# norabelrose/sparse-vae

Measured on AMD Instinct MI355X. Metric: training tokens/sec + ELBO match vs CPU ref, 512-tok seq, 1/2/4/8 MI355X, higher is better.
Workload: dtype bf16; 1 GPU; c2: TransformerVAE 6L d512 heads 8 seq 512, batch 64/GPU, dense attention, dropout 0.1, fwd+bwd+allreduce+clip+RAdam; model=TransformerVAE-6L-d512, global_batch=64, seq_len=512, parallelism=dp1

## Files before the change

### include/svae.h

```cpp
#ifndef SVAE_H
#define SVAE_H
#include <stdint.h>
#ifdef __cplusplus
extern "C" {
#endif

typedef void* svae_stream_t;

enum svae_epi {
  SVAE_EPI_BF16 = 0,
  SVAE_EPI_F32 = 1,
  SVAE_EPI_F32_ACC = 2,
  SVAE_EPI_F32_ATOMIC = 3,
  SVAE_EPI_GELU = 4,
  SVAE_EPI_GELU_BWD = 5,
  SVAE_EPI_DROPOUT_RESID = 6,
  SVAE_EPI_ROTARY_BF16 = 7,
  SVAE_EPI_CE_STATS = 8,
  SVAE_EPI_CE_PROB = 9,
  SVAE_EPI_ROWSCALE_GATHER = 10
};

typedef struct svae_gemm_desc {
  const void* A;
// ... 43 lines not shown
                      const float* zrows, int32_t zmod, const float* w, const float* b, float* xo, void* h, float* mean,
                      float* rstd, int32_t rows, int32_t D, svae_stream_t stream);
int svae_layernorm_fwd(const void* x, int32_t x_dtype, const float* w, const float* b, void* y,
                       float* mean, float* rstd, int32_t rows, int32_t D, svae_stream_t stream);
int svae_layernorm_bwd(const void* dy, const void* x, int32_t x_dtype, const float* w, const float* mean,
                       const float* rstd, const float* dres, float* dx, void* dx_bf, float* part,
                       int32_t nblk, int32_t rows, int32_t D, int32_t zero_mod, svae_stream_t stream);
int svae_layernorm_bwd_drop(const void* dy, const void* x, int32_t x_dtype, const float* w, const float* mean,
                            const float* rstd, const float* dres, float* dx, void* dx_bf, float* part, int32_t nblk,
                            int32_t rows, int32_t D, int32_t zero_mod, float bf_drop_p, uint64_t bf_seed,
                            int32_t bf_zero_mod, float* zrow, void* zrow_bf, svae_stream_t stream);
int svae_layernorm_bwd_gelu(const void* dy, const void* x, int32_t x_dtype, const float* w, const float* mean,
                            const float* rstd, const void* gp, void* out_bf, float* part, int32_t nblk, int32_t rows,
                            int32_t D, svae_stream_t stream);
int svae_layernorm_fwd_z(float* x, const float* zrows, int32_t zmod, const float* w, const float* b, void* y,
                         float* mean, float* rstd, int32_t rows, int32_t D, svae_stream_t stream);
int svae_layernorm_nblk(int32_t rows);
#define SVAE_LN_MULTI_MAX 4
int svae_layernorm_fwd_multi(const float* x, const float* const* w, const float* const* b, void* const* y, int32_t n,
                             float* mean, float* rstd, int32_t rows, int32_t D, svae_stream_t stream);
int svae_layernorm_bwd_multi(const void* const* dy, const float* x, const float* const* w, const float* mean,
                             const float* rstd, const float* dres, float* dx, float* const* part, int32_t nblk,
                             int32_t n, int32_t rows, int32_t D, svae_stream_t stream);

int svae_colsum(const void* in, int32_t in_dtype, int32_t rows, int32_t cols, int64_t ld, float* out,
                int32_t accumulate, svae_stream_t stream);

#define SVAE_COLSUM_MAX 8
typedef struct svae_colsum_seg {
  const float* in;
  float* out;
  int64_t ld;
  int32_t rows, cols;
} svae_colsum_seg;
int svae_colsum_multi(const svae_colsum_seg* segs, int32_t n, svae_stream_t stream);

typedef struct svae_attn_desc {
  const void* q; const void* k; const void* v; void* o;
  int64_t sq, sk, sv, so, bq, bk, bv, bo;
  const uint8_t* key_pad;
  float* lse;
  int32_t B, H, Lq, Lk, hd, causal;
  float scale;
  const void* dout; int64_t sdo, bdo;
  float* delta;
  float* dq;
// ... 247 lines not shown
```

### sparse-vae_amd/csrc/layernorm.hip

```cpp
#include <algorithm>

#include "common.h"
#include "../../include/svae.h"

using namespace svae;

namespace {


template <typename T>
__device__ __forceinline__ f32x4 load4(const T* p);
template <>
__device__ __forceinline__ f32x4 load4<float>(const float* p) { return *(const f32x4*)p; }
template <>
__device__ __forceinline__ f32x4 load4<bf16>(const bf16* p) {
  bf16x4 v = *(const bf16x4*)p;
  return (f32x4){(float)v[0], (float)v[1], (float)v[2], (float)v[3]};
}
__device__ __forceinline__ void store4_bf(bf16* p, f32x4 v) {
  *(bf16x4*)p = (bf16x4){f2bf(v[0]), f2bf(v[1]), f2bf(v[2]), f2bf(v[3])};
}

template <int MAXV>
__device__ __forceinline__ int ln_col(int lane, int k) {
// ... 426 lines not shown
    const float m1 = wave_sum(s1) / D, m2 = wave_sum(s2) / D;
#pragma unroll
    for (int j = 0; j < MAXV; ++j) {
      const int c = (lane + 64 * j) * 4;
      if (c < D) {
        f32x4 o;
#pragma unroll
        for (int e = 0; e < 4; ++e) o[e] = rstd * (g[j][e] - m1 - xh[j][e] * m2) + cur.rr[j][e];
        *(f32x4*)(dx + base + c) = o;
      }
    }
    cur = nxt;
  }
#pragma unroll
  for (int i = 0; i < NM; ++i) {
    if (i >= m.n) break;
    if (i > 0) __syncthreads();
#pragma unroll
    for (int j = 0; j < MAXV; ++j) {
      const int c = (lane + 64 * j) * 4;
      if (c < D) {
        *(f32x4*)&red[wave][0][c] = adw[i][j];
        *(f32x4*)&red[wave][1][c] = adb[i][j];
      }
    }
    __syncthreads();
    for (int c = threadIdx.x; c < 2 * D; c += 256) {
      const int which = c / D, col = c % D;
      const float s = red[0][which][col] + red[1][which][col] + red[2][which][col] + red[3][which][col];
      m.part[i][((long long)blockIdx.x * 2 + which) * D + col] = s;
    }
  }
}

template <typename T>
__global__ __launch_bounds__(256) void colsum_kernel(const T* __restrict__ in, int rows, int cols, long long ld,
                                                     float* __restrict__ out, int rows_per_split) {
  __shared__ f32x4 red[16][17];
  const int ct = threadIdx.x & 15, rt = threadIdx.x >> 4;
  const int c = (blockIdx.x * 16 + ct) * 4;
  const int r0 = blockIdx.y * rows_per_split;
  const int r1 = min(rows, r0 + rows_per_split);
  f32x4 acc = {0.f, 0.f, 0.f, 0.f};
  if (c < cols) {
    int r = r0 + rt;
    for (; r + 112 < r1; r += 128) {
// ... 196 lines not shown
  SVAE_LAUNCH_CHECK();
  return SVAE_OK;
}

SVAE_EXPORT int svae_layernorm_bwd_multi(const void* const* dy, const float* x, const float* const* w, const float* mean,
                                         const float* rstd, const float* dres, float* dx, float* const* part,
                                         int32_t nblk, int32_t n, int32_t rows, int32_t D, svae_stream_t stream) {
  if (!dy || !x || !w || !mean || !rstd || !dx || !part || n <= 0 || n > SVAE_LN_MULTI_MAX || rows <= 0 || D <= 0 ||
      D % 4 || D > 1024 || nblk <= 0)
    return SVAE_EINVAL;
  LnMulti m = {};
  m.n = n;
  for (int i = 0; i < n; ++i) {
    if (!dy[i] || !w[i] || !part[i]) return SVAE_EINVAL;
    m.dy[i] = (const bf16*)dy[i]; m.w[i] = w[i]; m.part[i] = part[i];
  }
  hipStream_t s = (hipStream_t)stream;
#define SVAE_LN_BWDM(MV) \
  hipLaunchKernelGGL((ln_bwd_multi_kernel<MV>), dim3(nblk), dim3(256), 0, s, m, x, mean, rstd, dres, dx, rows, D)
  if (D <= 512) SVAE_LN_BWDM(2);
  else if (D <= 768) SVAE_LN_BWDM(3);
  else SVAE_LN_BWDM(4);
#undef SVAE_LN_BWDM
  SVAE_LAUNCH_CHECK();
  return SVAE_OK;
}

SVAE_EXPORT int svae_layernorm_nblk(int32_t rows) {
  int n = (rows + 3) / 4;
  return n < 1024 ? n : 1024;
}

SVAE_EXPORT int svae_layernorm_bwd_drop(const void* dy, const void* x, int32_t x_dtype, const float* w,
                                        const float* mean, const float* rstd, const float* dres, float* dx, void* dx_bf,
                                        float* part, int32_t nblk, int32_t rows, int32_t D, int32_t zero_mod,
                                        float bf_drop_p, uint64_t bf_seed, int32_t bf_zero_mod, float* zrow,
                                        void* zrow_bf, svae_stream_t stream) {
  if (!dy || !x || !w || !mean || !rstd || !dx || !part || rows <= 0 || D <= 0 || D % 4 || D > 1024 || nblk <= 0)
    return SVAE_EINVAL;
  if (bf_drop_p < 0.f || bf_drop_p >= 1.f || ((bf_drop_p > 0.f || bf_zero_mod > 0) && !dx_bf)) return SVAE_EINVAL;
  if ((zrow || zrow_bf) && zero_mod <= 0) return SVAE_EINVAL;
  hipStream_t s = (hipStream_t)stream;
#define SVAE_LN_BWD(MV)                                                                                            \
  do {                                                                                                             \
    if (x_dtype == 0)                                                                                              \
      hipLaunchKernelGGL((ln_bwd_kernel<float, MV>), dim3(nblk), dim3(256), 0, s, (const bf16*)dy, (const float*)x, \
// ... 65 lines not shown
```

### sparse-vae_amd/sparse_vae/_native.py

```python
import ctypes
import os

import torch

_HERE = os.path.dirname(os.path.abspath(__file__))
LIB_PATH = os.environ.get('SVAE_LIB') or os.path.join(_HERE, 'libsvae.so')

c_void_p, c_int32, c_int64, c_float, c_uint64 = (ctypes.c_void_p, ctypes.c_int32, ctypes.c_int64,
                                                  ctypes.c_float, ctypes.c_uint64)
c_fptr = ctypes.c_void_p

EPI_BF16, EPI_F32, EPI_F32_ACC, EPI_F32_ATOMIC, EPI_GELU, EPI_GELU_BWD, EPI_DROPOUT_RESID, \
    EPI_ROTARY_BF16, EPI_CE_STATS, EPI_CE_PROB, EPI_ROWSCALE_GATHER = range(11)

LATENT_L2, LATENT_COSINE, LATENT_KL = range(3)
LATENT_METRICS = {'l2': LATENT_L2, 'cosine': LATENT_COSINE, 'kl': LATENT_KL}
LATENT_MAX_BLOCKS = 1024
TSNE_ROWS_PER_BLOCK, TSNE_TILE_COLS = 512, 256
PAIR_RBF, PAIR_IMQ = range(2)
PAIR_KINDS = {'rbf': PAIR_RBF, 'imq': PAIR_IMQ}
PAIRSUM_TILE_COLS, PAIRSUM_MAX_P, MMD_REDUCE_BLOCKS = 32, 8, 256
KMEANS_MAX_K, KMEANS_TILE_CENTROIDS, KMEANS_SORT_BLOCKS, KMEANS_SEED_BLOCK_ROWS = 1024, 32, 256, 256
TEXT_MAX_LEN = 2048
BEAM_MAX_W = 16
# ... 25 lines not shown
        ('q', c_void_p), ('k', c_void_p), ('v', c_void_p), ('o', c_void_p),
        ('sq', c_int64), ('sk', c_int64), ('sv', c_int64), ('so', c_int64),
        ('bq', c_int64), ('bk', c_int64), ('bv', c_int64), ('bo', c_int64),
        ('key_pad', c_void_p), ('lse', c_void_p),
        ('B', c_int32), ('H', c_int32), ('Lq', c_int32), ('Lk', c_int32), ('hd', c_int32), ('causal', c_int32),
        ('scale', c_float),
        ('dout', c_void_p), ('sdo', c_int64), ('bdo', c_int64),
        ('delta', c_void_p), ('dq', c_void_p), ('bdq', c_int64),
        ('dk', c_void_p), ('dv', c_void_p),
        ('sdk', c_int64), ('sdv', c_int64), ('bdk', c_int64), ('bdv', c_int64),
        ('rot_tab', c_void_p), ('rot_d', c_int32),
        ('o32', c_void_p), ('so32', c_int64), ('bo32', c_int64),
        ('dq_part', c_void_p), ('dq_bf', c_void_p), ('ldq_bf', c_int64),
        ('window', c_int32),
        ('delta_ready', c_int32),
        ('o_lo', c_void_p), ('so_lo', c_int64), ('bo_lo', c_int64),
        ('fwd_ws', c_void_p), ('fwd_ws_elems', c_int64),
    ]


GROUP_MAX = 256
COLSUM_MAX = 8
LN_MULTI_MAX = 4


ZPROJ_MAX = 32


class ZprojSeg(ctypes.Structure):
    _fields_ = [('g', c_void_p), ('W', c_void_p), ('dW', c_void_p), ('db', c_void_p)]


class ZprojFwdSeg(ctypes.Structure):
    _fields_ = [('W', c_void_p), ('bias', c_void_p), ('out', c_void_p)]


class ColsumSeg(ctypes.Structure):
    _fields_ = [('inp', c_void_p), ('out', c_void_p), ('ld', c_int64), ('rows', c_int32), ('cols', c_int32)]


_SIGS = {
    'svae_gemm': [ctypes.POINTER(GemmDesc), c_void_p],
    'svae_gemm_pair': [ctypes.POINTER(GemmDesc), ctypes.POINTER(GemmDesc), c_void_p],
    'svae_gemm_group_table_bytes': [c_int32],
    'svae_gemm_group': [ctypes.POINTER(GemmDesc), c_int32, c_int32, c_void_p, c_void_p, c_int64, c_void_p],
    'svae_resid_ln_fwd': [c_void_p, c_void_p, c_int32, c_int64, c_float, c_uint64, c_void_p, c_int32, c_void_p,
# ... 32 lines not shown
    'svae_ce_label_logit': [c_void_p, c_int64, c_void_p, c_int64, c_void_p, c_void_p, c_int32, c_int32, c_void_p,
                            c_void_p],
    'svae_ce_prob_finalize': [c_void_p, c_int32, c_void_p, c_void_p, c_int32, c_int32, c_int32, c_int32, c_void_p,
                              c_void_p, c_void_p, c_void_p, c_void_p, c_void_p],
    'svae_ce_prob_finalize_fix': [c_void_p, c_int32, c_void_p, c_void_p, c_int32, c_int32, c_int32, c_int32, c_void_p,
                                  c_void_p, c_void_p, c_void_p, c_void_p, c_void_p, c_int64, c_void_p, c_int64, c_void_p,
                                  c_void_p, c_int64, c_int32, c_int32, c_void_p, c_void_p],
    'svae_ce_prob_bwd_prep': [c_void_p, c_int64, c_void_p, c_void_p, c_void_p, c_void_p, c_void_p, c_int32, c_int32,
                              c_int32, c_int32, c_int32, c_void_p, c_void_p, c_void_p, c_void_p, c_void_p],
    'svae_embedding_bwd_ce': [c_void_p, c_void_p, c_void_p, c_int32, c_int32, c_int32, c_void_p, c_void_p, c_void_p],
    'svae_ce_grad': [c_void_p, c_int64, c_void_p, c_void_p, c_void_p, c_void_p, c_void_p, c_int32, c_int32, c_int32,
                     c_int32, c_int32, c_void_p],
    'svae_dropout_bwd_cast': [c_void_p, c_void_p, c_float, c_uint64, c_int64, c_int32, c_int64, c_void_p],
    'svae_gelu_bwd': [c_void_p, c_void_p, c_void_p, c_int64, c_void_p],
    'svae_prep_tokens': [c_void_p, c_void_p, c_int32, c_int32, c_int32, c_void_p, c_void_p, c_void_p, c_void_p,
                         c_void_p, c_void_p],
    'svae_step_scalars': [c_void_p, c_void_p, c_void_p, c_float, c_void_p, c_void_p, c_void_p],
    'svae_zproj_bwd_multi': [c_void_p, c_int32, c_void_p, c_void_p, c_int32, c_int32, c_int32, c_void_p],
    'svae_zproj_fwd_multi': [c_void_p, c_int32, c_void_p, c_int32, c_int32, c_int32, c_void_p],
    'svae_layernorm_fwd_multi': [c_void_p, c_void_p, c_void_p, c_void_p, c_int32, c_void_p, c_void_p, c_int32, c_int32,
                                 c_void_p],
    'svae_layernorm_bwd_multi': [c_void_p, c_void_p, c_void_p, c_void_p, c_void_p, c_void_p, c_void_p, c_void_p,
                                 c_int32, c_int32, c_int32, c_int32, c_void_p],
    'svae_layernorm_fwd_z': [c_void_p, c_void_p, c_int32, c_void_p, c_void_p, c_void_p, c_void_p, c_void_p, c_int32,
                             c_int32, c_void_p],
    'svae_cast_bf16': [c_void_p, c_void_p, c_int64, c_void_p],
    'svae_extract_rows': [c_void_p, c_int64, c_int32, c_int32, c_int32, c_void_p, c_void_p],
    'svae_zproj_bwd': [c_void_p, c_void_p, c_void_p, c_void_p, c_void_p, c_void_p, c_int32, c_int32, c_int32, c_void_p],
    'svae_sumsq': [c_void_p, c_int64, c_void_p, c_int32, c_void_p],
    'svae_radam': [c_void_p, c_void_p, c_void_p, c_void_p, c_void_p, c_int64, c_void_p, c_int32, c_void_p,
                   c_void_p, c_void_p],
    'svae_gemm_f32': [c_void_p, c_void_p, c_void_p, c_int32, c_int32, c_int32, c_int64, c_int64, c_int64, c_void_p,
                      c_void_p, c_int64, c_int32, c_void_p, c_int32, c_int32, c_int32, c_void_p],
    'svae_attn_fwd_f32': [c_void_p, c_void_p, c_void_p, c_void_p, c_int64, c_int64, c_int64, c_int64, c_int64, c_int64,
                          c_int64, c_int64, c_void_p, c_int32, c_int32, c_int32, c_int32, c_int32, c_int32, c_int32,
                          c_float, c_void_p],
    'svae_layernorm_fwd_f32': [c_void_p, c_void_p, c_void_p, c_void_p, c_int32, c_int32, c_void_p],
    'svae_ce_seq_logprob': [c_void_p, c_int32, c_void_p, c_void_p, c_int32, c_int32, c_void_p, c_void_p],
    'svae_dec_linear': [c_void_p, c_int64, c_void_p, c_int64, c_void_p, c_void_p, c_int64, c_void_p, c_int64, c_int32,
                        c_int32, c_int32, c_int32, c_void_p, c_int32, c_int32, c_void_p, c_void_p, c_int64, c_void_p],
    'svae_dec_attn': [c_void_p, c_int64, c_void_p, c_void_p, c_int32, c_int32, c_int32, c_int32, c_void_p, c_int32,
                      c_float, c_void_p, c_int64, c_void_p],
    'svae_dec_embed': [c_void_p, c_int32, c_void_p, c_void_p, c_void_p, c_int32, c_int32, c_void_p],
    'svae_dec_penalty': [c_void_p, c_int64, c_int32, c_void_p, c_void_p, c_int32, c_void_p, c_void_p, c_float,
                         c_void_p],
    'svae_dec_sample': [c_void_p, c_int64, c_int32, c_int32, c_void_p, c_void_p, c_int32, c_void_p, c_void_p, c_int32,
# ... 98 lines not shown
```

### sparse-vae_amd/sparse_vae/engine.py

```python
import math
import os
from collections import OrderedDict

import torch

from . import kernels as K
from ._native import COLSUM_MAX, GROUP_MAX, LN_MULTI_MAX, ZPROJ_MAX
from ._native import EPI_BF16, EPI_F32, EPI_F32_ACC, EPI_GELU, EPI_GELU_BWD, EPI_DROPOUT_RESID, \
    EPI_ROTARY_BF16, EPI_CE_STATS, EPI_F32_ATOMIC, EPI_CE_PROB, EPI_ROWSCALE_GATHER

bf16, f32 = torch.bfloat16, torch.float32
ALIGN = 64
CE_CHUNK_NUMEL = 2 ** 30


def _attn_entries(pre, d, learned):
    out = []
    if learned:
        out.append((pre + 'learned_queries', (1, learned, d)))
        names = ['k_linear', 'v_linear']
    else:
        names = ['q_linear', 'k_linear', 'v_linear']
    out += [(pre + n + '.weight', (d, d)) for n in names]
    out += [(pre + n + '.bias', (d,)) for n in names]
    out += [(pre + 'output_linear.weight', (d, d)), (pre + 'output_linear.bias', (d,))]
    return out


def _ctx_ln_entries(pre, d):
    return [(pre + 'context_layer_norm.weight', (d,)), (pre + 'context_layer_norm.bias', (d,))]
# ... 260 lines not shown

    def _bname(self, name, st):
        return f'{name}.{st["tag"]}' if self._dw_names else name

    def flush_dw(self):
        q, self._dw_jobs = self._dw_jobs, []
        k = 0
        for c in range(0, len(q), GROUP_MAX):
            jobs = q[c:c + GROUP_MAX]
            key = tuple((j.n_out, j.n_in, j.rows) for j in jobs)
            if key not in self._dwg_sched:
                self._dwg_sched[key] = K.group_schedule(key, self.ncu)
            for idx, splits, slab in self._dwg_sched[key]:
                if len(self._dwg_states) <= k:
                    self._dwg_states.append(K.DwGroupState(self.P.device))
                K.linear_dw_group([jobs[i] for i in idx], splits, self._dwg_states[k], slab=slab)
                k += 1

    def _db(self, dY, bname, rows, cols, ld=None):
        off = self.P.offsets[bname][0]
        K.colsum(dY, rows, cols, ld or cols, self.P.grad[off:off + cols])

    def layer_fwd(self, pre, x, B, Sx, L, pad, *, learned=0, cross=False, causal=False, ctx=None, heads, hd,
                  drop_p=0.0, seed=0, tag, out=None, window=0, out_bf=None, zsplice=None, ctx_ln=None):
        d, ws, P = self.d, self.ws, self.P
        rows_x = B * Sx
        rot = self.rot(max(Sx, L), window)
        st = {'pre': pre, 'B': B, 'Sx': Sx, 'L': L, 'learned': learned, 'cross': cross, 'causal': causal,
              'heads': heads, 'hd': hd, 'drop_p': drop_p, 'seed': seed, 'x': x, 'tag': tag, 'window': window}
        a = pre + 'attention.'
        h, st['ln_a'] = self._ln_fwd(pre + 'attn_layer_norm', x, rows_x, tag + '.ln_a', zsplice=zsplice)
        st['h'] = h
        pad_k = pad if Sx == L else None
        if learned:
            Lq = learned
            kv = ws.get(tag + '.kv', (rows_x, 2 * d))
            K.gemm(h, P.w(a + 'k_linear.weight'), kv, rows_x, 2 * d, d, epi=EPI_ROTARY_BF16,
                   bias=P.f(a + 'k_linear.bias'), rot=rot, rot_cols=d, rot_d=d, rot_seq=Sx)
            q = P.w(a + 'learned_queries').view(Lq, d)
            qargs = dict(sq=d, bq=0)
            kt, vt, sk = kv, kv[:, d:], 2 * d
            st['kv'] = kv
        else:
            Lq = Sx
            qkv = ws.get(tag + '.qkv', (rows_x, 3 * d))
            K.gemm(h, P.w(a + 'q_linear.weight'), qkv, rows_x, 3 * d, d, epi=EPI_ROTARY_BF16,
                   bias=P.f(a + 'q_linear.bias'), rot=rot, rot_cols=2 * d, rot_d=d, rot_seq=Sx)
            q = qkv
            qargs = dict(sq=3 * d, bq=Sx * 3 * d)
            kt, vt, sk = qkv[:, d:], qkv[:, 2 * d:], 3 * d
            st['qkv'] = qkv
        rows_q = B * Lq
        O = ws.get(tag + '.O', (rows_q, d))
        Ox = self._o_extra(tag + '.O', rows_q, d, Lq)
# ... 34 lines not shown
                   bias=P.f(c + 'output_linear.bias'), resid=x1, ldr=d)
            st.update(cx=cx, hq=hq, qc=qc, kvc=kvc, Oc=Oc, lsec=lsec, x2=x2, pad_ctx=pad)
            xc = x2
        h2, st['ln_f'] = self._ln_fwd(pre + 'ffn_layer_norm', xc, rows_q, tag + '.ln_f')
        gprime = ws.get(tag + '.gprime', (rows_q, 4 * d))
        f = ws.get(tag + '.f', (rows_q, 4 * d))
        K.gemm(h2, P.w(pre + 'ffn.0.weight'), f, rows_q, 4 * d, d, epi=EPI_GELU, bias=P.f(pre + 'ffn.0.bias'),
               aux=gprime, ldaux=4 * d)
        out = ws.get(tag + '.out', (rows_q, d), f32) if out is None else out
        K.gemm(f, P.w(pre + 'ffn.2.weight'), out, rows_q, d, 4 * d, epi=EPI_DROPOUT_RESID, resid=xc, ldr=d,
               drop_p=drop_p, seed=seed, aux=out_bf, ldaux=d if out_bf is not None else 0)
        st.update(h2=h2, gprime=gprime, f=f, xc=xc, rows_q=rows_q)
        return out, st

    def _o_extra(self, tag, rows_q, d, Lq):
        return dict(o_lo=self.ws.get(tag + 'lo', (rows_q, d)), so_lo=d, bo_lo=Lq * d)

    def _dq_part(self, B, H, Lq, Lk, hd, window=0):
        n = K.attn_dq_part_elems(B, H, Lq, Lk, hd, window)
        t = self.ws.bufs.get('b.dqpart')
        return t if t is not None and t.numel() >= n else self.ws.get('b.dqpart', (n,), f32)

    def layer_bwd(self, st, dout, dx_out, *, dx_accumulate=False, dctx=None, g2_ready=False, next_drop=None,
                  zsplice=None, next_st=None):
        d, ws, P = self.d, self.ws, self.P
        pre, B, Sx, L, Lq = st['pre'], st['B'], st['Sx'], st['L'], st['Lq']
        heads, hd = st['heads'], st['hd']
        rows_x, rows_q = B * Sx, st['rows_q']
        rot = self.rot(max(Sx, L), st['window'])
        a = pre + 'attention.'
        bn = lambda name: self._bname(name, st)
        self._dwq = self._dw_jobs if self._dw_names else None
        g2 = ws.get(bn('b.g2'), (rows_q, d))
        if not g2_ready:
            K.dropout_bwd_cast(dout, g2, st['drop_p'], st['seed'], rows_q, d)
        dpre = ws.get(bn('b.dpre'), (rows_q, 4 * d))
        K.gemm(g2, P.wT(pre + 'ffn.2.weight', d, 4 * d), dpre, rows_q, 4 * d, d, epi=EPI_GELU_BWD, aux=st['gprime'],
               ldaux=4 * d)
        self._dw_pair(self._job(g2, st['f'], pre + 'ffn.2.weight', rows_q, d, 4 * d),
                      self._job(dpre, st['h2'], pre + 'ffn.0.weight', rows_q, 4 * d, d, bias=pre + 'ffn.0.bias'))
        dh2 = ws.get('b.dh2', (rows_q, d))
        K.gemm(dpre, P.wT(pre + 'ffn.0.weight', 4 * d, d), dh2, rows_q, d, 4 * d, epi=EPI_BF16)
        dxc = ws.get('b.dxc', (rows_q, d), f32)
        gxc = ws.get(bn('b.gxc'), (rows_q, d))
        self._ln_bwd(pre + 'ffn_layer_norm', dh2, st['ln_f'], rows_q, dout, dxc, gxc)
        dx1, gx1 = dxc, gxc
        if st['cross']:
# ... 43 lines not shown
                                           bias=a + 'k_linear.bias'))
            dh = ws.get('b.dh', (rows_x, d))
            K.gemm(dkv, P.wT(a + 'k_linear.weight', 2 * d, d), dh, rows_x, d, 2 * d, epi=EPI_BF16)
        else:
            qkv = st['qkv']
            dqkv = ws.get(bn('b.dqkv'), (rows_x, 3 * d))
            K.attention(qkv, qkv[:, d:], qkv[:, 2 * d:], st['O'], st['lse'], B=B, H=heads, Lq=Lq, Lk=Sx, hd=hd,
                        sq=3 * d, bq=Sx * 3 * d, sk=3 * d, sv=3 * d, bk=Sx * 3 * d, bv=Sx * 3 * d, so=d, bo=Lq * d,
                        key_pad=st['pad_k'], causal=st['causal'], window=st['window'], backward=True, dout=dO,
                        sdo=d, bdo=Lq * d, delta=delta, dq_bf=dqkv, ldq_bf=3 * d, dk=dqkv[:, d:], dv=dqkv[:, 2 * d:],
                        sdk=3 * d, sdv=3 * d, bdk=Sx * 3 * d, bdv=Sx * 3 * d, rot=rot, rot_d=d, **st['Ox'],
                        dq_part=self._dq_part(B, heads, Lq, Sx, hd, st['window']))
            self._dw_pair(wo_dw, self._job(dqkv, st['h'], a + 'q_linear.weight', rows_x, 3 * d, d,
                                           bias=a + 'q_linear.bias'))
            dh = ws.get('b.dh', (rows_x, d))
            K.gemm(dqkv, P.wT(a + 'q_linear.weight', 3 * d, d), dh, rows_x, d, 3 * d, epi=EPI_BF16)
        if st['resid']:
            self._ln_bwd(pre + 'attn_layer_norm', dh, st['ln_a'], rows_x, dx1, dx_out,
                         dx_bf=(ws.get(self._bname('b.g2', next_st or st), (rows_x, d)) if next_drop is not None
                                else None), bf_drop=next_drop,
                         zsplice=zsplice)
            if dx_accumulate:
                raise NotImplementedError('residual + accumulate is handled by the caller')
        else:
            self._ln_bwd(pre + 'attn_layer_norm', dh, st['ln_a'], rows_x, dx_out if dx_accumulate else None, dx_out)
        self._dwq = None

    def forward(self, ids, ntok, *, pad=True, eps=None, seed=0, kl_weight=1.0, dropout=0.1, need_logits=False):
        hp, d, ws, P = self.hp, self.d, self.ws, self.P
        if not ids.is_cuda:
            raise RuntimeError('VAEEngine needs device tensors (no CPU fallback)')
        P.sync_shadow()
        B, L = ids.shape
        T, V, Z, N = B * L, hp.vocab_size, hp.latent_depth, hp.num_latents
        ids32 = ws.get('ids', (B, L), torch.int32)
        padm = None
        if pad is not None and pad is not False:
            padm = ws.get('pad', (B, L), torch.uint8)
        labels = ws.get('labels', (B, L), torch.int32)
        ntok64 = ws.get('ntok', (B,), torch.int64)
        if (ids.dtype == torch.int64 and ids.is_contiguous() and isinstance(ntok, torch.Tensor) and ntok.is_cuda
                and ntok.dtype == torch.int64 and ntok.is_contiguous() and ntok.numel() == B
                and (padm is None or pad is True or (pad.dtype == torch.bool and pad.is_contiguous()))):
            K.prep_tokens(ids, pad if padm is not None else None, B, L, ids32, labels, padm, ntok, ntok64)
        else:
            ids32, padm = self._inputs(ids, pad)
            labels[:, :-1].copy_(ids32[:, 1:])
            labels[:, -1] = 0
            ntok64.copy_(ntok)
        sv = {'B': B, 'L': L, 'dropout': dropout, 'seed': seed}

        x_emb = ws.get('x_emb', (T, d), f32)
        K.embedding_fwd(ids32, P.f('input_layer.0.weight'), x_emb, T, d, out2=ws.get('x_dec0', (T, d), f32))

        enc_bf, stats, sv['enc_layers'] = self._encode(x_emb, B, L, padm, dropout, seed)

        zf = ws.get('z', (B, Z), f32)
        zb = ws.get('z_bf', (B, Z))
        eps_buf = ws.get('eps', (B, Z), f32)
        raw_kl = ws.get('raw_kl', (B,), f32)
        kl = ws.get('kl', (2,), f32)
        if eps is not None:
            eps_buf.copy_(eps.reshape(B, Z))
        K.reparam_fwd(stats, eps_buf if eps is not None else None, _mix_seed(seed, 7), ntok64, zf, zb, eps_buf,
                      raw_kl, kl, B, Z)
        sv.update(enc_bf=enc_bf, stats=stats, z_bf=zb, eps=eps_buf)

        xf, sv['dec_layers'] = self._decode(x_emb, zb, padm, B, L, dropout, seed, x_ready=True)

        hh, gp0, h0, ln_h = self._head_hidden(xf, T)
        nchunks, chunk_len = K.ce_chunking(B, L, V, CE_CHUNK_NUMEL)
        lse = ws.get('ce.lse', (T,), f32)
        row_loss = ws.get('ce.row_loss', (T,), f32)
        chunk_w = ws.get('ce.chunk_w', (max(8, nchunks),), f32)
        nll = ws.get('nll', (1,), f32)
        ntile = -(-V // 128)
        head = 'logits' if need_logits else self.head_mode
        W, bias = P.w('input_layer.0.weight'), P.f('output_layer.3.bias')
# ... 20 lines not shown
            sat = ws.get('ce.sat', (T + 1,), torch.int32)
            K.ce_prob_finalize(part, ntile, coff, labels, T, L, nchunks, chunk_len, lse, row_loss, chunk_w, nll,
                               fix=(hh, W, bias, logits, sat))
        else:
            K.ce_finalize(part, ntile, lab_logit, labels, T, L, nchunks, chunk_len, lse, row_loss, chunk_w, nll)
        sv.update(xf=xf, gp0=gp0, h0=h0, hh=hh, ln_h=ln_h, logits=logits, lse=lse, chunk_w=chunk_w,
                  nchunks=nchunks, chunk_len=chunk_len, labels=labels, ids32=ids32, ntok=ntok64, x_emb=x_emb,
                  row_loss=row_loss, head=head, coff=coff)
        loss = ws.get('loss', (1,), f32)
        K.step_scalars(kl_weight, nll=nll, kl=kl, loss=loss)
        self.saved = sv
        return {'loss': loss[0], 'nll': nll[0], 'kl': kl[0], 'train_kl': kl[1], 'raw_kl': raw_kl,
                'mu': stats[:, :Z], 'logvar': stats[:, Z:], 'stats': stats, 'kl_buf': kl, 'z': zf, 'eps': eps_buf,
                'logits': logits if need_logits else None,
                'ce_saturated': sat[0] if head == 'prob' else None}

    def weighted_nll(self, tok_w):
        sv = self.saved
        out = torch.empty(1, dtype=f32, device=self.P.device)
        B, L = sv['B'], sv['L']
        K.ce_weighted_nll(sv['row_loss'], sv['labels'], tok_w, B * L, L, sv['nchunks'], sv['chunk_len'], out)
        return out[0]

    def _encode(self, x_emb, B, L, padm, dropout, seed):
        hp, d, ws, P = self.hp, self.d, self.ws, self.P
        N, Z = hp.num_latents, hp.latent_depth
        lay = []
        z, st = self.layer_fwd('encoder.first_layer.', x_emb, B, L, L, padm, learned=N, heads=self.He, hd=64,
                               drop_p=dropout, seed=_mix_seed(seed, 1000), tag='e0')
        lay.append(st)
        nmid = hp.enc_layers - 2
        cxs = self._ctx_ln_fwd(x_emb, B * L, nmid) if P.ctx_batched else [None] * nmid
        for j in range(nmid):
            z, st = self.layer_fwd(f'encoder.middle_layers.{j}.', z, B, N, L, padm, cross=True, ctx=x_emb,
                                   heads=self.He, hd=64, drop_p=dropout, seed=_mix_seed(seed, 1001 + j), tag=f'e{j + 1}',
                                   ctx_ln=cxs[j])
            lay.append(st)
        enc, st = self.layer_fwd('encoder.bottleneck.', z, B, N, L, padm, learned=1, heads=self.He, hd=64,
                                 drop_p=dropout, seed=_mix_seed(seed, 1999), tag='eb')
        lay.append(st)
        enc_bf = ws.get('enc_bf', (B, d))
        K.cast_bf16(enc, enc_bf)
        stats = ws.get('stats', (B, 2 * Z), f32)
        K.gemm(enc_bf, P.w('q_of_z_given_x.linear.weight'), stats, B, 2 * Z, d, epi=EPI_F32,
               bias=P.f('q_of_z_given_x.linear.bias'))
        return enc_bf, stats, lay

    def _ctx_ln_fwd(self, x, rows, nmid):
        D, ws, P = self.d, self.ws, self.P
        mean = ws.get('ctx.ln.mean', (rows,), f32)
        rstd = ws.get('ctx.ln.rstd', (rows,), f32)
        out = []
        for j0 in range(0, nmid, LN_MULTI_MAX):
            js = range(j0, min(nmid, j0 + LN_MULTI_MAX))
            names = [f'encoder.middle_layers.{j}.context_layer_norm' for j in js]
# ... 273 lines not shown
                self._zp_pending.append((dzh_i, P.w(wz), P.g(wz), P.g(bz)))
            else:
                self.flush_zproj()
                K.extract_rows(dx_prev, d, T, L, d, dzh)
                K.cast_bf16(dzh, dzh_bf)
                self._dw(self._job(dzh_bf, sv['z_bf'], wz, B, d, Z, bias=bz))
                K.gemm(dzh_bf, P.w(wz), dz, B, Z, d, b_t=True, epi=EPI_F32_ATOMIC, splits=max(1, min(8, d // 64)))
            ready(P.end(f'z_projections.{i}.bias'))
            dx, dx_prev = dx_prev, dx
        self.flush_zproj()
        dx_emb = dx

        dstats = ws.get('b.dstats', (B, 2 * Z), f32)
        K.reparam_bwd(sv['stats'], sv['eps'], dz, sv['ntok'], gs[1:2], dstats, B, Z)
        dstats_bf = ws.get('b.dstats_bf', (B, 2 * Z))
        K.cast_bf16(dstats, dstats_bf)
        self._dw(self._job(dstats_bf, sv['enc_bf'], 'q_of_z_given_x.linear.weight', B, 2 * Z, d))
        self._db(dstats, 'q_of_z_given_x.linear.bias', B, 2 * Z)
        denc = ws.get('b.denc', (B, d), f32)
        K.gemm(dstats_bf, P.w('q_of_z_given_x.linear.weight'), denc, B, d, 2 * Z, b_t=True, epi=EPI_F32)
        ready(P.end('q_of_z_given_x.linear.bias'))

        enc = sv['enc_layers']
        dcur = denc
        for k in reversed(range(1, len(enc))):
            st = enc[k]
            nxt = ws.get(f'b.denc{k}', (B * N, d), f32)
            self.layer_bwd(st, dcur, nxt, dctx=dx_emb)
            ready(P.end(st['pre'] + 'ffn_layer_norm.bias'))
            dcur = nxt
        deferred = [st for st in enc if st.get('ctx_deferred')]
        if deferred:
            self._ctx_ln_bwd(deferred[::-1], dx_emb)
            ready(P.end(deferred[0]['pre'] + 'context_layer_norm.bias'))
        st0 = enc[0]
        if st0['resid']:
            tmp = ws.get('b.dfirst', (T, d), f32)
            self.layer_bwd(st0, dcur, tmp)
            self.flush_dw()
            K.embedding_bwd(sv['ids32'], tmp, P.g('input_layer.0.weight'), T, d)
        else:
            self.layer_bwd(st0, dcur, dx_emb, dx_accumulate=True)
            self.flush_dw()

        ready(P.end('encoder.first_layer.ffn_layer_norm.bias'))
        self._embedding_bwd(sv, dx_emb, T, d)
        ready(P.n_live)
        self.flush_colsum()

    def _embedding_bwd(self, sv, dx, T, d):
        if sv['head'] == 'prob':
            K.embedding_bwd_ce(sv['ids32'], dx, self.P.g('input_layer.0.weight'), T, d, sv['L'], sv['hh'], sv['ce_q'])
        else:
            K.embedding_bwd(sv['ids32'], dx, self.P.g('input_layer.0.weight'), T, d)
```

### sparse-vae_amd/sparse_vae/kernels.py

```python
import ctypes
import os
from typing import NamedTuple

import torch

from . import _native as N
from ._native import lib, check, ptr, stream

bf16, f32 = torch.bfloat16, torch.float32

_gemm_desc = N.GemmDesc()


def _dev(*ts):
    for t in ts:
        if t is not None and not t.is_cuda:
            raise RuntimeError('libsvae kernels need device tensors (no CPU fallback)')


def gemm(A, B, C, M, N_, K, *, a_t=False, b_t=False, lda=None, ldb=None, ldc=None, epi=N.EPI_BF16, bias=None,
         resid=None, ldr=0, aux=None, ldaux=0, alpha=1.0, splits=1, drop_p=0.0, seed=0, rot=None, rot_cols=0,
         rot_d=0, rot_seq=0, labels=None, label_logit=None, batch=1, sA=0, sB=0, sC=0, a_rowsum=None, k_weight=None,
         row_a=None, row_b=None, gather=None, ldg=0, delta=None, delta_o32=None, ld_o32=0, delta_hd=0, delta_seq=0):
    d = _fill_desc(_gemm_desc, A, B, C, M, N_, K, a_t=a_t, b_t=b_t, lda=lda, ldb=ldb, ldc=ldc, epi=epi, bias=bias,
# ... 279 lines not shown

def _ptrs(ts):
    return (ctypes.c_void_p * N.LN_MULTI_MAX)(*[t.data_ptr() for t in ts])


def layernorm_fwd_multi(x, ws, bs, ys, mean, rstd, rows, D):
    n = len(ys)
    assert 0 < n <= N.LN_MULTI_MAX and len(ws) == n and len(bs) == n and x.dtype == f32
    _dev(x, mean, rstd, *ws, *bs, *ys)
    check(lib.svae_layernorm_fwd_multi(x.data_ptr(), _ptrs(ws), _ptrs(bs), _ptrs(ys), n, mean.data_ptr(),
                                       rstd.data_ptr(), rows, D, stream()), 'svae_layernorm_fwd_multi')


def layernorm_bwd_multi(dys, x, ws, mean, rstd, dres, dx, wgrads, rows, D, part_ws, defer=None):
    n = len(dys)
    assert 0 < n <= N.LN_MULTI_MAX and len(ws) == n and len(wgrads) == n and x.dtype == f32
    _dev(x, mean, rstd, dx, *dys, *ws)
    nblk = lib.svae_layernorm_nblk(rows)
    parts = [part_ws[j * nblk * 2 * D:(j + 1) * nblk * 2 * D] for j in range(n)]
    assert parts[-1].numel() == nblk * 2 * D
    check(lib.svae_layernorm_bwd_multi(_ptrs(dys), x.data_ptr(), _ptrs(ws), mean.data_ptr(), rstd.data_ptr(),
                                       ptr(dres), dx.data_ptr(), _ptrs(parts), nblk, n, rows, D, stream()),
          'svae_layernorm_bwd_multi')
    for part, wg in zip(parts, wgrads):
        if defer is not None:
            defer.append((part, nblk, 2 * D, 2 * D, wg))
        else:
            colsum(part, nblk, 2 * D, 2 * D, wg, accumulate=True)


_colsum_segs = (N.ColsumSeg * N.COLSUM_MAX)()


def colsum_multi(segs):
    assert 0 < len(segs) <= N.COLSUM_MAX
    for i, (inp, rows, cols, ld, out) in enumerate(segs):
        _dev(inp, out)
        assert inp.dtype == f32 and out.dtype == f32
        _colsum_segs[i].inp, _colsum_segs[i].out = inp.data_ptr(), out.data_ptr()
        _colsum_segs[i].ld, _colsum_segs[i].rows, _colsum_segs[i].cols = ld, rows, cols
    check(lib.svae_colsum_multi(ctypes.addressof(_colsum_segs), len(segs), stream()), 'svae_colsum_multi')


def colsum(inp, rows, cols, ld, out, accumulate=True):
    check(lib.svae_colsum(inp.data_ptr(), 0 if inp.dtype == f32 else 1, rows, cols, ld, out.data_ptr(),
                          int(accumulate), stream()), 'svae_colsum')
# ... 817 lines not shown
```

Baseline: 2.826 million tokens/s.

## Fuse embedding gather with encoder layernorms in forward and backward

Adds a kernel that gathers embedding rows and in one pass computes the shared layernorm statistics and writes the bf16 normalized outputs for the first layer's attention LN and the middle layers' context LNs. A matching backward kernel folds those layernorm backwards, including weight/bias partial sums, into the embedding scatter-add. This removes separate embedding and LN launches and extra round trips of the T×d activations through memory. In exchange it adds more complex gradient-readiness ordering for the allreduce and per-element atomics into the embedding table in the fused backward.

```diff
diff --git a/include/svae.h b/include/svae.h
--- a/include/svae.h
+++ b/include/svae.h
@@ -89,6 +89,14 @@
 int svae_layernorm_bwd_multi(const void* const* dy, const float* x, const float* const* w, const float* mean,
                              const float* rstd, const float* dres, float* dx, float* const* part, int32_t nblk,
                              int32_t n, int32_t rows, int32_t D, svae_stream_t stream);
+#define SVAE_EMB_LN_MAX (SVAE_LN_MULTI_MAX + 1)
+int svae_embedding_ln_fwd_multi(const int32_t* ids, const void* table, const float* const* w, const float* const* b,
+                                void* const* y, int32_t n, float* out, float* out2, float* mean, float* rstd,
+                                int32_t rows, int32_t D, svae_stream_t stream);
+int svae_embedding_bwd_ln_multi(const int32_t* ids, const float* dx, const float* x, const float* mean,
+                                const float* rstd, const void* const* dy, const float* const* w, float* const* part,
+                                int32_t nblk, int32_t n, float* dtable, int32_t rows, int32_t D, int32_t seq,
+                                const void* hh, const float* q, svae_stream_t stream);
 
 int svae_colsum(const void* in, int32_t in_dtype, int32_t rows, int32_t cols, int64_t ld, float* out,
                 int32_t accumulate, svae_stream_t stream);
diff --git a/sparse-vae_amd/csrc/layernorm.hip b/sparse-vae_amd/csrc/layernorm.hip
--- a/sparse-vae_amd/csrc/layernorm.hip
+++ b/sparse-vae_amd/csrc/layernorm.hip
@@ -472,6 +472,166 @@
       if (c < D) {
         *(f32x4*)&red[wave][0][c] = adw[i][j];
         *(f32x4*)&red[wave][1][c] = adb[i][j];
+      }
+    }
+    __syncthreads();
+    for (int c = threadIdx.x; c < 2 * D; c += 256) {
+      const int which = c / D, col = c % D;
+      const float s = red[0][which][col] + red[1][which][col] + red[2][which][col] + red[3][which][col];
+      m.part[i][((long long)blockIdx.x * 2 + which) * D + col] = s;
+    }
+  }
+}
+
+struct EmbLn {
+  const float* w[SVAE_EMB_LN_MAX];
+  const float* b[SVAE_EMB_LN_MAX];
+  bf16* y[SVAE_EMB_LN_MAX];
+  const bf16* dy[SVAE_EMB_LN_MAX];
+  float* part[SVAE_EMB_LN_MAX];
+  int n;
+};
+
+template <int MAXV>
+__global__ __launch_bounds__(256) void emb_ln_fwd_multi_kernel(const int* __restrict__ ids,
+                                                               const float* __restrict__ table, EmbLn m,
+                                                               float* __restrict__ out, float* __restrict__ out2,
+                                                               float* __restrict__ mean_out,
+                                                               float* __restrict__ rstd_out, int rows, int D) {
+  const int lane = threadIdx.x & 63;
+  const int nw = gridDim.x * 4;
+  int row = blockIdx.x * 4 + (threadIdx.x >> 6);
+  if (row >= rows) return;
+  f32x4 v[MAXV], vn[MAXV];
+  ln_load_row<float, MAXV>(table + (long long)ids[row] * D, lane, D, v);
+#pragma nounroll
+  while (true) {
+    const int next = row + nw;
+    if (next < rows) ln_load_row<float, MAXV>(table + (long long)ids[next] * D, lane, D, vn);
+#pragma unroll
+    for (int k = 0; k < MAXV; ++k) {
+      const int c = ln_col<MAXV>(lane, k);
+      if (c < D) {
+        *(f32x4*)(out + (long long)row * D + c) = v[k];
+        *(f32x4*)(out2 + (long long)row * D + c) = v[k];
+      }
+    }
+    float s = 0.f;
+#pragma unroll
+    for (int k = 0; k < MAXV; ++k) s += (v[k][0] + v[k][1]) + (v[k][2] + v[k][3]);
+    const float mean = wave_sum(s) / D;
+    float sq = 0.f;
+#pragma unroll
+    for (int k = 0; k < MAXV; ++k) {
+      const bool in = ln_col<MAXV>(lane, k) < D;
+#pragma unroll
+      for (int e = 0; e < 4; ++e) { const float t = in ? v[k][e] - mean : 0.f; sq += t * t; }
+    }
+    const float rstd = rsqrtf(wave_sum(sq) / D + 1e-5f);
+#pragma unroll
+    for (int j = 0; j < SVAE_EMB_LN_MAX; ++j)
+      if (j < m.n) ln_store_row<MAXV>(v, mean, rstd, m.w[j], m.b[j], m.y[j] + (long long)row * D, lane, D);
+    if (lane == 0) { mean_out[row] = mean; rstd_out[row] = rstd; }
+    if (next >= rows) break;
+    for (int k = 0; k < MAXV; ++k) v[k] = vn[k];
+    row = next;
+  }
+}
+
+template <int NK, int NM>
+__global__ __launch_bounds__(256) void emb_bwd_ln_multi_kernel(const int* __restrict__ ids, EmbLn m,
+                                                               const float* __restrict__ dx,
+                                                               const float* __restrict__ x,
+                                                               const float* __restrict__ mean_in,
+                                                               const float* __restrict__ rstd_in,
+                                                               float* __restrict__ dtable, int rows, int D, int seq,
+                                                               const bf16* __restrict__ hh,
+                                                               const float* __restrict__ q) {
+  __shared__ float red[4][2][64 * NK];
+  const int lane = threadIdx.x & 63, wave = threadIdx.x >> 6;
+  float adw[NM][NK], adb[NM][NK];
+#pragma unroll
+  for (int i = 0; i < NM; ++i)
+#pragma unroll
+    for (int k = 0; k < NK; ++k) { adw[i][k] = 0.f; adb[i][k] = 0.f; }
+  struct RowIn {
+    float xv[NK], rr[NK];
+    bf16 dv[NM][NK], hv[NK];
+    float mean, rstd, qp;
+    long long dst;
+  };
+  auto load_row = [&](int row, RowIn& in) {
+    const long long base = (long long)row * D;
+    in.mean = mean_in[row];
+    in.rstd = rstd_in[row];
+    in.dst = (long long)ids[row] * D;
+    const bool head = hh && row % seq != 0;
+    in.qp = head ? q[row - 1] : 0.f;
+#pragma unroll
+    for (int k = 0; k < NK; ++k) {
+      const int c = lane + 64 * k;
+      const bool ok = c < D;
+      in.xv[k] = ok ? x[base + c] : 0.f;
+      in.rr[k] = ok ? dx[base + c] : 0.f;
+      in.hv[k] = ok && head ? hh[base - D + c] : (bf16)0.f;
+#pragma unroll
+      for (int i = 0; i < NM; ++i) {
+        if (i >= m.n) break;
+        in.dv[i][k] = ok ? m.dy[i][base + c] : (bf16)0.f;
+      }
+    }
+  };
+  const int stride = gridDim.x * 4;
+  int row = blockIdx.x * 4 + wave;
+  RowIn cur, nxt;
+  if (row < rows) load_row(row, cur);
+  for (; row < rows; row += stride) {
+    if (row + stride < rows) load_row(row + stride, nxt);
+    const float mean = cur.mean, rstd = cur.rstd, qp = cur.qp;
+    const long long dst = cur.dst;
+    float xh[NK], g[NK], r[NK];
+    float s1 = 0.f, s2 = 0.f;
+#pragma unroll
+    for (int k = 0; k < NK; ++k) {
+      const int c = lane + 64 * k;
+      g[k] = 0.f; xh[k] = 0.f; r[k] = 0.f;
+      if (c < D) {
+        xh[k] = (cur.xv[k] - mean) * rstd;
+        r[k] = cur.rr[k];
+#pragma unroll
+        for (int i = 0; i < NM; ++i) {
+          if (i >= m.n) break;
+          const float dv = (float)cur.dv[i][k];
+          g[k] += dv * m.w[i][c];
+          adw[i][k] = __builtin_fmaf(dv, xh[k], adw[i][k]);
+          adb[i][k] += dv;
+        }
+        s1 += g[k];
+        s2 += g[k] * xh[k];
+      }
+    }
+    const float m1 = wave_sum(s1) / D, m2 = wave_sum(s2) / D;
+#pragma unroll
+    for (int k = 0; k < NK; ++k) {
+      const int c = lane + 64 * k;
+      if (c < D) {
+        float o = rstd * (g[k] - m1 - xh[k] * m2) + r[k];
+        if (qp != 0.f) o -= qp * (float)cur.hv[k];
+        atomicAdd(dtable + dst + c, o);
+      }
+    }
+    cur = nxt;
+  }
+#pragma unroll
+  for (int i = 0; i < NM; ++i) {
+    if (i >= m.n) break;
+    if (i > 0) __syncthreads();
+#pragma unroll
+    for (int k = 0; k < NK; ++k) {
+      const int c = lane + 64 * k;
+      if (c < D) {
+        red[wave][0][c] = adw[i][k];
+        red[wave][1][c] = adb[i][k];
       }
     }
     __syncthreads();
@@ -714,6 +874,68 @@
   else if (D <= 768) SVAE_LN_BWDM(3);
   else SVAE_LN_BWDM(4);
 #undef SVAE_LN_BWDM
+  SVAE_LAUNCH_CHECK();
+  return SVAE_OK;
+}
+
+SVAE_EXPORT int svae_embedding_ln_fwd_multi(const int32_t* ids, const void* table, const float* const* w,
+                                            const float* const* b, void* const* y, int32_t n, float* out, float* out2,
+                                            float* mean, float* rstd, int32_t rows, int32_t D, svae_stream_t stream) {
+  if (!ids || !table || !w || !b || !y || !out || !out2 || !mean || !rstd || n <= 0 || n > SVAE_EMB_LN_MAX ||
+      rows <= 0 || D <= 0 || D % 4 || D > 1024)
+    return SVAE_EINVAL;
+  if (((uintptr_t)table | (uintptr_t)out | (uintptr_t)out2) & 15) return SVAE_EINVAL;
+  EmbLn m = {};
+  m.n = n;
+  for (int i = 0; i < n; ++i) {
+    if (!w[i] || !b[i] || !y[i]) return SVAE_EINVAL;
+    m.w[i] = w[i]; m.b[i] = b[i]; m.y[i] = (bf16*)y[i];
+  }
+  const LnFwdPlan plan = ln_fwd_plan(rows, D);
+  const dim3 grid(plan.grid);
+  hipStream_t s = (hipStream_t)stream;
+#define SVAE_EMB_LN_FWD(MV)                                                                                      \
+  hipLaunchKernelGGL((emb_ln_fwd_multi_kernel<MV>), grid, dim3(256), 0, s, ids, (const float*)table, m, out, out2, \
+                     mean, rstd, rows, D)
+  if (plan.mv == 2) SVAE_EMB_LN_FWD(2);
+  else if (plan.mv == 3) SVAE_EMB_LN_FWD(3);
+  else if (plan.mv == 4) SVAE_EMB_LN_FWD(4);
+  else SVAE_EMB_LN_FWD(5);
+#undef SVAE_EMB_LN_FWD
+  SVAE_LAUNCH_CHECK();
+  return SVAE_OK;
+}
+
+SVAE_EXPORT int svae_embedding_bwd_ln_multi(const int32_t* ids, const float* dx, const float* x, const float* mean,
+                                            const float* rstd, const void* const* dy, const float* const* w,
+                                            float* const* part, int32_t nblk, int32_t n, float* dtable, int32_t rows,
+                                            int32_t D, int32_t seq, const void* hh, const float* q,
+                                            svae_stream_t stream) {
+  if (!ids || !dx || !x || !mean || !rstd || !dy || !w || !part || !dtable || n <= 0 || n > SVAE_EMB_LN_MAX ||
+      rows <= 0 || D <= 0 || D % 4 || D > 768 || nblk <= 0)
+    return SVAE_EINVAL;
+  if ((hh == nullptr) != (q == nullptr) || (hh && (seq <= 0 || rows % seq))) return SVAE_EINVAL;
+  EmbLn m = {};
+  m.n = n;
+  for (int i = 0; i < n; ++i) {
+    if (!dy[i] || !w[i] || !part[i]) return SVAE_EINVAL;
+    m.dy[i] = (const bf16*)dy[i]; m.w[i] = w[i]; m.part[i] = part[i];
+  }
+  hipStream_t s = (hipStream_t)stream;
+#define SVAE_EMB_BWD_LN(NK)                                                                                        \
+  do {                                                                                                             \
+    if (n <= 2)                                                                                                    \
+      hipLaunchKernelGGL((emb_bwd_ln_multi_kernel<NK, 2>), dim3(nblk), dim3(256), 0, s, ids, m, dx, x, mean, rstd, \
+                         dtable, rows, D, seq > 0 ? seq : 1, (const bf16*)hh, q);                                  \
+    else                                                                                                           \
+      hipLaunchKernelGGL((emb_bwd_ln_multi_kernel<NK, SVAE_EMB_LN_MAX>), dim3(nblk), dim3(256), 0, s, ids, m, dx,  \
+                         x, mean, rstd, dtable, rows, D, seq > 0 ? seq : 1, (const bf16*)hh, q);                   \
+  } while (0)
+  if (D <= 128) SVAE_EMB_BWD_LN(2);
+  else if (D <= 256) SVAE_EMB_BWD_LN(4);
+  else if (D <= 512) SVAE_EMB_BWD_LN(8);
+  else SVAE_EMB_BWD_LN(12);
+#undef SVAE_EMB_BWD_LN
   SVAE_LAUNCH_CHECK();
   return SVAE_OK;
 }
diff --git a/sparse-vae_amd/sparse_vae/_native.py b/sparse-vae_amd/sparse_vae/_native.py
--- a/sparse-vae_amd/sparse_vae/_native.py
+++ b/sparse-vae_amd/sparse_vae/_native.py
@@ -71,6 +71,7 @@
 GROUP_MAX = 256
 COLSUM_MAX = 8
 LN_MULTI_MAX = 4
+EMB_LN_MAX = LN_MULTI_MAX + 1
 
 
 ZPROJ_MAX = 32
@@ -149,6 +150,11 @@
                                  c_void_p],
     'svae_layernorm_bwd_multi': [c_void_p, c_void_p, c_void_p, c_void_p, c_void_p, c_void_p, c_void_p, c_void_p,
                                  c_int32, c_int32, c_int32, c_int32, c_void_p],
+    'svae_embedding_ln_fwd_multi': [c_void_p, c_void_p, c_void_p, c_void_p, c_void_p, c_int32, c_void_p, c_void_p,
+                                    c_void_p, c_void_p, c_int32, c_int32, c_void_p],
+    'svae_embedding_bwd_ln_multi': [c_void_p, c_void_p, c_void_p, c_void_p, c_void_p, c_void_p, c_void_p, c_void_p,
+                                    c_int32, c_int32, c_void_p, c_int32, c_int32, c_int32, c_void_p, c_void_p,
+                                    c_void_p],
     'svae_layernorm_fwd_z': [c_void_p, c_void_p, c_int32, c_void_p, c_void_p, c_void_p, c_void_p, c_void_p, c_int32,
                              c_int32, c_void_p],
     'svae_cast_bf16': [c_void_p, c_void_p, c_int64, c_void_p],
diff --git a/sparse-vae_amd/sparse_vae/engine.py b/sparse-vae_amd/sparse_vae/engine.py
--- a/sparse-vae_amd/sparse_vae/engine.py
+++ b/sparse-vae_amd/sparse_vae/engine.py
@@ -5,7 +5,7 @@
 import torch
 
 from . import kernels as K
-from ._native import COLSUM_MAX, GROUP_MAX, LN_MULTI_MAX, ZPROJ_MAX
+from ._native import COLSUM_MAX, EMB_LN_MAX, GROUP_MAX, LN_MULTI_MAX, ZPROJ_MAX
 from ._native import EPI_BF16, EPI_F32, EPI_F32_ACC, EPI_GELU, EPI_GELU_BWD, EPI_DROPOUT_RESID, \
     EPI_ROTARY_BF16, EPI_CE_STATS, EPI_F32_ATOMIC, EPI_CE_PROB, EPI_ROWSCALE_GATHER
 
@@ -312,14 +312,17 @@
         K.colsum(dY, rows, cols, ld or cols, self.P.grad[off:off + cols])
 
     def layer_fwd(self, pre, x, B, Sx, L, pad, *, learned=0, cross=False, causal=False, ctx=None, heads, hd,
-                  drop_p=0.0, seed=0, tag, out=None, window=0, out_bf=None, zsplice=None, ctx_ln=None):
+                  drop_p=0.0, seed=0, tag, out=None, window=0, out_bf=None, zsplice=None, ctx_ln=None, attn_ln=None):
         d, ws, P = self.d, self.ws, self.P
         rows_x = B * Sx
         rot = self.rot(max(Sx, L), window)
         st = {'pre': pre, 'B': B, 'Sx': Sx, 'L': L, 'learned': learned, 'cross': cross, 'causal': causal,
               'heads': heads, 'hd': hd, 'drop_p': drop_p, 'seed': seed, 'x': x, 'tag': tag, 'window': window}
         a = pre + 'attention.'
-        h, st['ln_a'] = self._ln_fwd(pre + 'attn_layer_norm', x, rows_x, tag + '.ln_a', zsplice=zsplice)
+        if attn_ln is not None:
+            h, st['ln_a'] = attn_ln
+        else:
+            h, st['ln_a'] = self._ln_fwd(pre + 'attn_layer_norm', x, rows_x, tag + '.ln_a', zsplice=zsplice)
         st['h'] = h
         pad_k = pad if Sx == L else None
         if learned:
@@ -400,7 +403,7 @@
         return t if t is not None and t.numel() >= n else self.ws.get('b.dqpart', (n,), f32)
 
     def layer_bwd(self, st, dout, dx_out, *, dx_accumulate=False, dctx=None, g2_ready=False, next_drop=None,
-                  zsplice=None, next_st=None):
+                  zsplice=None, next_st=None, skip_attn_ln=False):
         d, ws, P = self.d, self.ws, self.P
         pre, B, Sx, L, Lq = st['pre'], st['B'], st['Sx'], st['L'], st['Lq']
         heads, hd = st['heads'], st['hd']
@@ -490,6 +493,8 @@
                          zsplice=zsplice)
             if dx_accumulate:
                 raise NotImplementedError('residual + accumulate is handled by the caller')
+        elif skip_attn_ln:
+            st['dh'] = dh
         else:
             self._ln_bwd(pre + 'attn_layer_norm', dh, st['ln_a'], rows_x, dx_out if dx_accumulate else None, dx_out)
         self._dwq = None
@@ -519,9 +524,12 @@
         sv = {'B': B, 'L': L, 'dropout': dropout, 'seed': seed}
 
         x_emb = ws.get('x_emb', (T, d), f32)
-        K.embedding_fwd(ids32, P.f('input_layer.0.weight'), x_emb, T, d, out2=ws.get('x_dec0', (T, d), f32))
-
-        enc_bf, stats, sv['enc_layers'] = self._encode(x_emb, B, L, padm, dropout, seed)
+        sv['emb_fused'] = fused = self._emb_ln_fused(L)
+        if not fused:
+            K.embedding_fwd(ids32, P.f('input_layer.0.weight'), x_emb, T, d, out2=ws.get('x_dec0', (T, d), f32))
+
+        enc_bf, stats, sv['enc_layers'] = self._encode(x_emb, B, L, padm, dropout, seed,
+                                                       gather=ids32 if fused else None)
 
         zf = ws.get('z', (B, Z), f32)
         zb = ws.get('z_bf', (B, Z))
@@ -588,15 +596,35 @@
         K.ce_weighted_nll(sv['row_loss'], sv['labels'], tok_w, B * L, L, sv['nchunks'], sv['chunk_len'], out)
         return out[0]
 
-    def _encode(self, x_emb, B, L, padm, dropout, seed):
+    def _emb_ln_fused(self, L):
+        nmid = self.hp.enc_layers - 2
+        assert EMB_LN_MAX >= 2
+        return L != self.hp.num_latents and 0 <= nmid <= 1 and K.embedding_ln_supported(self.d)
+
+    def _encode(self, x_emb, B, L, padm, dropout, seed, gather=None):
         hp, d, ws, P = self.hp, self.d, self.ws, self.P
         N, Z = hp.num_latents, hp.latent_depth
         lay = []
+        nmid = hp.enc_layers - 2
+        attn_ln = None
+        if gather is not None:
+            rows = B * L
+            names = ['encoder.first_layer.attn_layer_norm']
+            names += [f'encoder.middle_layers.{j}.context_layer_norm' for j in range(nmid)]
+            ys = [ws.get('e0.ln_a.y', (rows, d))] + [ws.get(f'e{j + 1}.ln_ctx.y', (rows, d)) for j in range(nmid)]
+            mean = ws.get('emb.ln.mean', (rows,), f32)
+            rstd = ws.get('emb.ln.rstd', (rows,), f32)
+            K.embedding_ln_fwd_multi(gather, P.f('input_layer.0.weight'), [P.f(n + '.weight') for n in names],
+                                     [P.f(n + '.bias') for n in names], ys, x_emb, ws.get('x_dec0', (rows, d), f32),
+                                     mean, rstd, rows, d)
+            saved = (x_emb, mean, rstd)
+            attn_ln = (ys[0], saved)
+            cxs = [(y, saved) for y in ys[1:]]
         z, st = self.layer_fwd('encoder.first_layer.', x_emb, B, L, L, padm, learned=N, heads=self.He, hd=64,
-                               drop_p=dropout, seed=_mix_seed(seed, 1000), tag='e0')
+                               drop_p=dropout, seed=_mix_seed(seed, 1000), tag='e0', attn_ln=attn_ln)
         lay.append(st)
-        nmid = hp.enc_layers - 2
-        cxs = self._ctx_ln_fwd(x_emb, B * L, nmid) if P.ctx_batched else [None] * nmid
+        if gather is None:
+            cxs = self._ctx_ln_fwd(x_emb, B * L, nmid) if P.ctx_batched else [None] * nmid
         for j in range(nmid):
             z, st = self.layer_fwd(f'encoder.middle_layers.{j}.', z, B, N, L, padm, cross=True, ctx=x_emb,
                                    heads=self.He, hd=64, drop_p=dropout, seed=_mix_seed(seed, 1001 + j), tag=f'e{j + 1}',
@@ -916,18 +944,36 @@
         ready(P.end('q_of_z_given_x.linear.bias'))
 
         enc = sv['enc_layers']
+        fused = sv['emb_fused']
+        late = []
         dcur = denc
         for k in reversed(range(1, len(enc))):
             st = enc[k]
             nxt = ws.get(f'b.denc{k}', (B * N, d), f32)
             self.layer_bwd(st, dcur, nxt, dctx=dx_emb)
-            ready(P.end(st['pre'] + 'ffn_layer_norm.bias'))
+            end = P.end(st['pre'] + 'ffn_layer_norm.bias')
+            if late or (fused and st.get('ctx_deferred') and not P.ctx_batched):
+                late.append(end)
+            else:
+                ready(end)
             dcur = nxt
         deferred = [st for st in enc if st.get('ctx_deferred')]
+        st0 = enc[0]
+        if fused:
+            self.layer_bwd(st0, dcur, None, skip_attn_ln=True)
+            self.flush_dw()
+            self._embedding_bwd_ln(sv, dx_emb, deferred[::-1] + [st0], T, d)
+            for end in late:
+                ready(end)
+            if deferred and P.ctx_batched:
+                ready(P.end(deferred[0]['pre'] + 'context_layer_norm.bias'))
+            ready(P.end('encoder.first_layer.ffn_layer_norm.bias'))
+            ready(P.n_live)
+            self.flush_colsum()
+            return
         if deferred:
             self._ctx_ln_bwd(deferred[::-1], dx_emb)
             ready(P.end(deferred[0]['pre'] + 'context_layer_norm.bias'))
-        st0 = enc[0]
         if st0['resid']:
             tmp = ws.get('b.dfirst', (T, d), f32)
             self.layer_bwd(st0, dcur, tmp)
@@ -942,6 +988,23 @@
         ready(P.n_live)
         self.flush_colsum()
 
+    def _embedding_bwd_ln(self, sv, dx, sts, T, d):
+        P = self.P
+        names = [g['pre'] + ('context_layer_norm' if g['cross'] else 'attn_layer_norm') for g in sts]
+        dys = [g['dcx'] if g['cross'] else g['dh'] for g in sts]
+        x, mean, rstd = sts[-1]['ln_a']
+        wgs = [P.grad[P.offsets[n + '.weight'][0]:][:2 * d] for n in names]
+        n1 = 1024 * 2 * d
+        if len(self._cs_pending) + len(sts) > COLSUM_MAX:
+            self.flush_colsum()
+        k = len(self._cs_pending)
+        part = self.ws.get('ln.parts', (COLSUM_MAX * n1,), f32)[k * n1:(k + len(sts)) * n1]
+        prob = sv['head'] == 'prob'
+        K.embedding_bwd_ln_multi(sv['ids32'], dx, x, mean, rstd, dys, [P.f(n + '.weight') for n in names], wgs,
+                                 P.g('input_layer.0.weight'), T, d, part, seq=sv['L'] if prob else 0,
+                                 hh=sv['hh'] if prob else None, q=sv['ce_q'] if prob else None,
+                                 defer=self._cs_pending)
+
     def _embedding_bwd(self, sv, dx, T, d):
         if sv['head'] == 'prob':
             K.embedding_bwd_ce(sv['ids32'], dx, self.P.g('input_layer.0.weight'), T, d, sv['L'], sv['hh'], sv['ce_q'])
diff --git a/sparse-vae_amd/sparse_vae/kernels.py b/sparse-vae_amd/sparse_vae/kernels.py
--- a/sparse-vae_amd/sparse_vae/kernels.py
+++ b/sparse-vae_amd/sparse_vae/kernels.py
@@ -325,6 +325,43 @@
     check(lib.svae_layernorm_bwd_multi(_ptrs(dys), x.data_ptr(), _ptrs(ws), mean.data_ptr(), rstd.data_ptr(),
                                        ptr(dres), dx.data_ptr(), _ptrs(parts), nblk, n, rows, D, stream()),
           'svae_layernorm_bwd_multi')
+    for part, wg in zip(parts, wgrads):
+        if defer is not None:
+            defer.append((part, nblk, 2 * D, 2 * D, wg))
+        else:
+            colsum(part, nblk, 2 * D, 2 * D, wg, accumulate=True)
+
+
+def _emb_ptrs(ts):
+    return (ctypes.c_void_p * N.EMB_LN_MAX)(*[t.data_ptr() for t in ts])
+
+
+def embedding_ln_supported(D):
+    return D % 4 == 0 and 0 < D <= 768
+
+
+def embedding_ln_fwd_multi(ids, table, ws, bs, ys, out, out2, mean, rstd, rows, D):
+    n = len(ys)
+    assert 0 < n <= N.EMB_LN_MAX and len(ws) == n and len(bs) == n and table.dtype == f32
+    _dev(ids, table, out, out2, mean, rstd, *ws, *bs, *ys)
+    check(lib.svae_embedding_ln_fwd_multi(ids.data_ptr(), table.data_ptr(), _emb_ptrs(ws), _emb_ptrs(bs),
+                                          _emb_ptrs(ys), n, out.data_ptr(), out2.data_ptr(), mean.data_ptr(),
+                                          rstd.data_ptr(), rows, D, stream()), 'svae_embedding_ln_fwd_multi')
+
+
+def embedding_bwd_ln_multi(ids, dx, x, mean, rstd, dys, ws, wgrads, dtable, rows, D, part_ws, seq=0, hh=None, q=None,
+                           defer=None):
+    n = len(dys)
+    assert 0 < n <= N.EMB_LN_MAX and len(ws) == n and len(wgrads) == n and x.dtype == f32 and dx.dtype == f32
+    assert (hh is None) == (q is None)
+    _dev(ids, dx, x, mean, rstd, dtable, *dys, *ws)
+    nblk = lib.svae_layernorm_nblk(rows)
+    parts = [part_ws[j * nblk * 2 * D:(j + 1) * nblk * 2 * D] for j in range(n)]
+    assert parts[-1].numel() == nblk * 2 * D
+    check(lib.svae_embedding_bwd_ln_multi(ids.data_ptr(), dx.data_ptr(), x.data_ptr(), mean.data_ptr(),
+                                          rstd.data_ptr(), _emb_ptrs(dys), _emb_ptrs(ws), _emb_ptrs(parts), nblk, n,
+                                          dtable.data_ptr(), rows, D, int(seq), ptr(hh), ptr(q), stream()),
+          'svae_embedding_bwd_ln_multi')
     for part, wg in zip(parts, wgrads):
         if defer is not None:
             defer.append((part, nblk, 2 * D, 2 * D, wg))
```

Result: no change. 2.838 million tokens/s (median of 6 runs) (+0.4%).
